# QData/FastSK

Hardware: AMD Instinct MI355X
Metric: gkm kernel build: mismatch-combos/s (higher is better)
Workload: dtype u4 count planes (v_dot8_u32_u4), u32 register sums, u64 triangle (plain stores on the first pass over reset rows, else atomics); 1 GPU; config5: synthetic DNA 100000 x 300 bp, g=12 m=8 exact, 495 combos; n_seq=100000, seq_len=300, g=12, m=8, combos=495, parallelism=single GPU

## Files before the change

### fastsk_amd/csrc/fsk_engine_dense_shift.hip

```cpp
#include "fsk_engine_internal.h"
#include "fsk_kernels_dense_shift.h"

#include <map>

using namespace fsk_detail;

namespace fsk {

#define FSK_DMA_SHIFT 1
#define FSK_DMA_KERNEL k_dense_tile_shift
#define FSK_DMA_COMPACT 0
#include "fsk_tile_kernel_dma.inc"
#undef FSK_DMA_KERNEL
#undef FSK_DMA_COMPACT
#undef FSK_DMA_SHIFT

}

namespace fsk_detail {

bool dense_shift_plan(fsk_engine* e, const int32_t* combos, int n, u64 by_overflow, uint32_t max_chain) {
    ShiftPlan& p = e->shift;
    if (!(p.by_overflow == by_overflow && p.max_chain == max_chain && (int)p.combos.size() == n && std::equal(combos, combos + n, p.combos.begin()))) {
        p = ShiftPlan();
        p.combos.assign(combos, combos + n);
        p.by_overflow = by_overflow;
        p.max_chain = max_chain;
        const int k = e->k;
        std::map<std::vector<uint8_t>, std::vector<std::pair<int, int>>> shapes;
        for (int q = 0; q < n; ++q) {
            const uint8_t* pos = &e->all_pos[(size_t)combos[q] * k];
            std::vector<uint8_t> shape(pos, pos + k);
            for (auto& x : shape) x = (uint8_t)(x - pos[0]);
            shapes[shape].push_back({(int)pos[0], q});
        }
        std::vector<std::vector<int>> chains;
        for (auto& kv : shapes) {
            auto& v = kv.second;
            std::stable_sort(v.begin(), v.end(), [](const std::pair<int, int>& a, const std::pair<int, int>& b) { return a.first < b.first; });
            for (size_t i = 0; i < v.size(); ++i) {
                if (i == 0 || v[i].first != v[i - 1].first + 1 || (max_chain != 0u && chains.back().size() >= max_chain)) chains.emplace_back();
                chains.back().push_back(v[i].second);
            }
        }
        std::stable_sort(chains.begin(), chains.end(), [](const std::vector<int>& a, const std::vector<int>& b) { return a.size() > b.size(); });
        p.n_bases = (uint32_t)chains.size();
        p.order.resize((size_t)n);
        uint32_t derived = p.n_bases;
        size_t group_begin = 0;
        for (size_t c = 0; c < chains.size(); ++c) {
            const std::vector<int>& ch = chains[c];
            const uint32_t len = (uint32_t)ch.size();
            p.order[c] = ch[0];
            if (c == 0 || chains[c - 1].size() != ch.size() || (u64)(c - group_begin) >= by_overflow) {
                p.groups.push_back(0u);
                p.groups.push_back(len);
                group_begin = c;
            }
            p.groups[p.groups.size() - 2] = (uint32_t)c + 1u;
            uint32_t lower = (uint32_t)c;
            for (uint32_t u = 1; u < len; ++u) {
                const uint32_t upper = derived++;
                p.order[upper] = ch[u];
                p.steps.push_back(upper << 16 | lower);
                p.steps.push_back(len - u);
                p.wsum += len - u;
                lower = upper;
            }
        }
    }
    return !p.steps.empty() && n <= 32768 && ((u64)2 * e->maxW + 32) * p.wsum < ((u64)1 << 31);
}

int dense_shift_edge_keys(fsk_engine* e, const uint8_t* chunk_pos, uint32_t panels_pad) {
    ShiftPlan& p = e->shift;
    const uint32_t n_steps = (uint32_t)(p.steps.size() / 2), np_seq = panels_pad * fsk::PANEL;
    FSK_HIP(e->d_shift_steps.reserve(p.steps.size()));
    FSK_HIP(e->d_edge_keys.reserve((size_t)n_steps * np_seq));
    FSK_HIP(hipMemcpyAsync(e->d_shift_steps.p, p.steps.data(), p.steps.size() * sizeof(uint32_t), hipMemcpyHostToDevice, e->stream));
    FSK_LAUNCH(fsk::k_dense_edge_keys, dim3(panels_pad, (n_steps + 3u) / 4u), dim3(256), 0, e->stream, e->view(), e->cfg.g, e->k, e->sigma, chunk_pos,
               (const uint32_t*)e->d_shift_steps.p, n_steps, np_seq, e->d_edge_keys.p);
    FSK_HIP(hipStreamSynchronize(e->stream));
    e->st.launches += 1;
    return FSK_OK;
}

int dense_shift_keymajor(fsk_engine* e, uint32_t panels_pad, int nb, uint32_t Vq8) {
    const ShiftPlan& p = e->shift;
    e->ld.shift_packed = false;
    if (e->tune.dense_shift_packed < 0 || p.max_chain != SHIFT_PACKED_CHAIN) return FSK_OK;
    const size_t plane = (size_t)panels_pad * Vq8 * fsk::PANEL * (size_t)nb;
    const size_t n_keys = (p.steps.size() / 2) * (size_t)panels_pad * fsk::PANEL;
    const size_t want = (2 * plane + n_keys) * sizeof(uint32_t);
    const char* why = nullptr;
    if (e->tune.dense_shift_plane_kb > 0 && want > (size_t)e->tune.dense_shift_plane_kb * 1024) why = "over the dense_shift_plane_kb cap";
    const size_t grow = (std::max(plane, e->d_KM.cap) - e->d_KM.cap + std::max(plane, e->d_KMH.cap) - e->d_KMH.cap +
                         std::max(n_keys, e->d_edge_offs.cap) - e->d_edge_offs.cap) * sizeof(uint32_t);
    if (!why && grow > 0) {
        size_t free_b = 0, total_b = 0;
        if (hipMemGetInfo(&free_b, &total_b) != hipSuccess) free_b = 0;
        if (grow > free_b / 2) why = "more than half of the free device memory";
        else if (e->d_KM.reserve(plane) != hipSuccess || e->d_KMH.reserve(plane) != hipSuccess || e->d_edge_offs.reserve(n_keys) != hipSuccess) {
            (void)hipGetLastError();
            e->d_KM.release(); e->d_KMH.release(); e->d_edge_offs.release();
            why = "hipMalloc failed";
        }
    }
    if (why) {
        if (e->trace())
            fprintf(stderr, "[fsk] dense shift classes: the key-major planes (%.1f MB) do not fit, %s: k_dense_shift_fix runs the corrections\n",
                    (double)want / 1e6, why);
        return FSK_OK;
    }
    const uint32_t n_pairs = panels_pad / 2u;
    const uint32_t kgrid = (uint32_t)(((size_t)n_pairs * nb * Vq8 * 16u + 255u) / 256u);
    FSK_LAUNCH(fsk::k_dense_keymajor, dim3(kgrid), dim3(256), 0, e->stream, (const uint32_t*)e->d_C4.p, n_pairs, nb, Vq8, e->d_KM.p);
    FSK_LAUNCH(fsk::k_dense_keymajor, dim3(kgrid), dim3(256), 0, e->stream, (const uint32_t*)e->d_C4H.p, n_pairs, nb, Vq8, e->d_KMH.p);
    FSK_LAUNCH(fsk::k_dense_edge_offs, dim3((uint32_t)((n_keys + 255u) / 256u)), dim3(256), 0, e->stream, (const uint16_t*)e->d_edge_keys.p, n_keys,
               e->d_edge_offs.p);
    e->st.launches += 3;
    e->ld.shift_packed = true;
    return FSK_OK;
}

int dense_shift_tiles(fsk_engine* e, u64 n_tiles, int nb, uint32_t Vq8, uint32_t nst, u64* K, int store, uint32_t panels_pad) {
    const ShiftPlan& p = e->shift;
    int slot0 = 0;
    for (size_t gi = 0; gi + 1 < p.groups.size(); gi += 2) {
        const int end = (int)p.groups[gi];
        FSK_LAUNCH(fsk::k_dense_tile_shift, dim3((uint32_t)n_tiles, 1), dim3(256), 0, e->stream, (const uint32_t*)e->d_C4.p, (const uint32_t*)e->d_C4H.p,
                   (const uint32_t*)e->d_rowmask.p, (const uint32_t*)e->d_tiletab.p, nb, Vq8, nst, (uint32_t)e->N, K, end - slot0, gi == 0 ? store : 0,
                   slot0, p.groups[gi + 1]);
        slot0 = end;
    }
    if (e->ld.shift_packed) {
        const auto k_packed = e->tune.dense_shift_inplace != 0 ? fsk::k_dense_shift_packed<true> : fsk::k_dense_shift_packed<false>;
        FSK_LAUNCH(k_packed, dim3((uint32_t)n_tiles), dim3(256), 0, e->stream, (const uint32_t*)e->d_KM.p, (const uint32_t*)e->d_KMH.p,
                   (const uint32_t*)e->d_rowmask.p, (const uint32_t*)e->d_tiletab.p, (const uint32_t*)e->d_shift_steps.p, (uint32_t)(p.steps.size() / 2),
                   (const uint32_t*)e->d_edge_offs.p, panels_pad * fsk::PANEL, nb, Vq8, p.n_bases, (uint32_t)(32u * p.wsum), (uint32_t)e->N, K);
    } else {
        FSK_LAUNCH(fsk::k_dense_shift_fix, dim3((uint32_t)n_tiles), dim3(512), 0, e->stream, (const uint32_t*)e->d_C4.p, (const uint32_t*)e->d_C4H.p,
                   (const uint32_t*)e->d_rowmask.p, (const uint32_t*)e->d_tiletab.p, (const uint32_t*)e->d_shift_steps.p, (uint32_t)(p.steps.size() / 2),
                   (const uint16_t*)e->d_edge_keys.p, panels_pad * fsk::PANEL, nb, Vq8, (uint32_t)e->N, K);
    }
    e->st.launches += (int32_t)(p.groups.size() / 2);
    return FSK_OK;
}

}
```

### fastsk_amd/csrc/fsk_engine_internal.h

```cpp
#pragma once
#include "fsk_common.h"

#include <algorithm>
#include <chrono>
#include <cmath>
#include <cstdarg>
#include <cstdio>
#include <cstdlib>
#include <cstring>
#include <string>
#include <array>
#include <atomic>
#include <thread>
#include <vector>

#include <cstdint>
#include <climits>

#include "../../include/fastsk_amd.h"
#include <condition_variable>
#include <functional>
#include <memory>
#include <mutex>

struct fsk_group;

namespace fsk_detail {

#define FSK_HIP(call)                                                                          \
    do {                                                                                       \
        hipError_t _e = (call);                                                                \
        if (_e != hipSuccess) return e->fail(FSK_EDEVICE, "%s failed: %s", #call, hipGetErrorString(_e)); \
    } while (0)

template <typename T>
struct DevBuf {
    T* p = nullptr;
    size_t cap = 0;
    DevBuf() = default;
    DevBuf(DevBuf&& o) noexcept : p(o.p), cap(o.cap) { o.p = nullptr; o.cap = 0; }
    DevBuf& operator=(DevBuf&& o) noexcept { std::swap(p, o.p); std::swap(cap, o.cap); return *this; }
    ~DevBuf() { release(); }
    hipError_t reserve(size_t n) {
        if (n <= cap) return hipSuccess;
        release();
        hipError_t r = hipMalloc((void**)&p, n * sizeof(T));
        if (r == hipSuccess) cap = n;
        return r;
    }
    void release() {
        if (p) (void)hipFree(p);
        p = nullptr;
        cap = 0;
    }
};

template <typename T>
struct PinnedBuf {
    T* p = nullptr;
    size_t cap = 0;
    PinnedBuf() = default;
    PinnedBuf(PinnedBuf&& o) noexcept : p(o.p), cap(o.cap) { o.p = nullptr; o.cap = 0; }
    PinnedBuf& operator=(PinnedBuf&& o) noexcept { std::swap(p, o.p); std::swap(cap, o.cap); return *this; }
    ~PinnedBuf() { release(); }
    hipError_t reserve(size_t n, size_t slack = 0) {
        if (n <= cap) return hipSuccess;
        release();
        hipError_t r = hipHostMalloc((void**)&p, (n + slack) * sizeof(T));
        if (r == hipSuccess) cap = n + slack;
        return r;
    }
    void release() {
        if (p) (void)hipHostFree(p);
        p = nullptr;
        cap = 0;
    }
};

template <typename H, hipError_t (*Create)(H*, unsigned), hipError_t (*Destroy)(H)>
struct Handle {
    H h = nullptr;
    Handle() = default;
    Handle(Handle&& o) noexcept : h(o.h) { o.h = nullptr; }
    Handle& operator=(Handle&& o) noexcept { std::swap(h, o.h); return *this; }
    ~Handle() { if (h) (void)Destroy(h); }
    hipError_t create(unsigned flags) { return h ? hipSuccess : Create(&h, flags); }
    operator H() const { return h; }
};
using Stream = Handle<hipStream_t, hipStreamCreateWithFlags, hipStreamDestroy>;
using Event = Handle<hipEvent_t, hipEventCreateWithFlags, hipEventDestroy>;

struct DeviceScope {
    int prev = -1, dev;
    hipError_t err = hipSuccess;
    explicit DeviceScope(int d) : dev(d) {
        if (hipGetDevice(&prev) != hipSuccess) prev = -1;
        if (prev != dev) err = hipSetDevice(dev);
    }
    ~DeviceScope() {
        if (prev >= 0 && prev != dev) (void)hipSetDevice(prev);
    }
    DeviceScope(const DeviceScope&) = delete;
    DeviceScope& operator=(const DeviceScope&) = delete;
};
#define FSK_ON_DEVICE(e)                                                                      \
    DeviceScope fsk_on_device_((e)->cfg.device);                                             \
    if (fsk_on_device_.err != hipSuccess)                                                    \
        return (e)->fail(FSK_EDEVICE, "hipSetDevice(%d) failed: %s", (e)->cfg.device, hipGetErrorString(fsk_on_device_.err))

}

using fsk_detail::DevBuf;
using fsk_detail::PinnedBuf;
using fsk_detail::Stream;
using fsk_detail::Event;

#define FSK_TUNING_KEYS(X)                                                                                                          \
    X(trace, 0, 0, 1, "stderr: the tuning in force, where the host time of a load and of a variance-mode call goes")                 \
    X(profile, -1, -1, 2, "fsk_config.profile from here on (-1: as the engine was created)")                                          \
    X(compact, -1, -1, 1, "dense: key compaction off / on whatever the alphabet says (-1: a rare symbol decides)")                   \
    X(compact_rare, -1, -1, 1, "dense: keys that occur from the places of the rare symbols (1) or a marking pass over every window (0)") \
    X(tile_splits, 0, 0, 4096, "dense: combo splits per tile (0: by the size of the launch)")                                        \
    X(dense_small, 0, 0, 1, "dense: 1 = a split tile launch (small N) leaves its sums as 32-bit staging blocks that k_dense_widen adds into K (0: one 64-bit atomic a cell and split — measured faster: the atomics drain under other workgroups' dot products)")                                        \
    X(dense_shift, 0, -1, 1, "dense: one weighted Gram product per chain of shifted combinations, the other members by edge lookups (fsk_engine_dense_shift.hip) — 1 = whenever the call is eligible, -1 = never (0: when eligible, tile_splits = 0 and the launch has 16384 tiles or more, the size from which a tile has one workgroup anyway)") \
    X(dense_shift_packed, 0, -1, 0, "dense, shift classes: the derived steps from key-major planes, eight cells an LDS read (k_dense_keymajor, k_dense_shift_packed; chains cut at nine members) — 0 = whenever the shift path runs and the planes fit, -1 = never: k_dense_shift_fix on the count panels") \
    X(dense_shift_inplace, 1, 0, 1, "dense, shift classes: k_dense_shift_packed stages a chain's first planes and makes every further step's in LDS, one nibble up and one down a sequence (a step that meets a count above 15 in its tile, and the step behind it, are staged) — 0 = every step staged") \
    X(dense_shift_plane_kb, 0, 0, (int64_t)1 << 40, "dense, shift classes: the key-major planes and offsets may take this many KiB at most (0: half of the free memory; tests: the planes do not fit)") \
    X(dense_chunk, 0, 0, 1 << 24, "dense: cap of the count kernel's staging chunk, in windows (0: none)")                             \
    X(variance_dense_slots, 1, 0, 1, "variance mode, dense: 0 = zero fill + k_welford per iteration instead of storing slot triangles") \
    X(var_slots16, 1, 0, 1, "variance mode, sparse: 0 = u32 slot triangles from the start")                                          \
    X(sparse_global, 0, 0, 1, "sparse: every += as a 64-bit atomicAdd (k_sx_emit<DIRECT>) whatever N is")                             \
    X(sparse_unpacked, 0, 0, 1, "sparse: entries in the general 8 + 4 (+ 4) byte format whatever N is")                               \
    X(sparse_pairs, 1, 0, 1, "sparse: 0 = every update word 32 bits wide (1: unit products of clean runs travel two to a word)")      \
    X(sparse_sync, 0, 0, 1, "sparse: wait for every batch's word count and size its stream exactly")                                 \
    X(sparse_hint, 1, 0, 1, "sparse: 0 = the words per record of the previous set of sequences are never kept as a hint")             \
    X(sparse_exact_lanes, 0, 0, 2, "sparse: the batches of an exact accumulate never (1) / always (2) in two lanes (0: from six batches on)") \
    X(sparse_batch_records, 0, 0, (int64_t)1 << 31, "sparse: records per batch at most (0: 2^27)")                                   \
    X(guard_cap, 0, 0, (int64_t)1 << 40, "sparse: pretend the stream buffer holds this many words (0: its real size)")                \
    X(list_max_words, 0, 0, (int64_t)1 << 31, "sparse: update words of one batch beyond which its pairs go to K with atomics (0: 2^31)") \
    X(seg_scan_chunked, 0, 0, 1, "sparse: the three-launch segment scan whatever the tile count")                                    \
    X(extract_slots, 0, 0, 4, "sparse: slots per k_sx_extract_win workgroup, 1 or 4 (0: by the size of the launch)")                  \
    X(sparse_form, 0, 0, 3, "sparse: the update stage — 1 = owner bands whenever they exist, 2 = two-level blocks, 3 = 64-bit atomics (0: bands up to four LDS rounds a band, blocks beyond)") \
    X(blocks_sub_shift, 14, 4, 14, "sparse, blocks: log2 of the cells one k_sxb_consume workgroup sums in LDS (tests: small blocks on small inputs)") \
    X(blocks_max_bands, 512, 2, 512, "sparse, blocks: bands of one pass at most (tests: several passes on small inputs)")            \
    X(blocks_band_shift_max, 23, 4, 23, "sparse, blocks: log2 of a band's cells at most (tests)")                                    \
    X(blocks_pass_words, 0, 0, (int64_t)1 << 32, "sparse, blocks: update words of one pass at most (0: 2^31)")                       \
    X(sparse_desc, 0, -1, 1, "sparse, owner bands and two-level blocks: entries of many partners leave k_sx_emit as descriptors (one an entry; blocks: one per sub-band its partners fall into) that k_sx_consume / k_sxb_consume expand in LDS — 1 = always, -1 = never (0: once a batch of these sequences has shown sparse_desc_from pairs per record)") \
    X(sparse_desc_blocks, 1, 0, 1, "sparse, two-level blocks: 0 = never descriptors there (1: as sparse_desc says — one record per sub-band an entry's partners fall into)") \
    X(sparse_desc_cols, 1, 0, 3, "sparse, descriptors: where the partners are read from — 0 = the entries themselves; 1 = a column array (sequence id | multiplicity, 4 bytes) beside 8-byte entries, the entries themselves when they are packed (measured: 2-byte columns beside packed entries are no faster, 0.88 against 0.84 s in the large-g regime; 4-byte columns beside 8-byte entries 4.69 -> 4.44 ms a combo at N = 100k); tests: 2 = 4-byte columns always, 3 = 2-byte columns when N < 32768") \
    X(sparse_desc_min, 16, 1, 48, "sparse, descriptors: entries of more partners than this become descriptors (48: everything k_sx_emit does not bin in LDS; measured, large-g regime: 48 0.92 s, 32 0.85, 16 0.83-0.85, 8 0.88, 4 0.90)") \
    X(sparse_desc_from, 12, 1, 1 << 20, "sparse, descriptors: the pairs per sort record of a batch from which on the following batches use them (sparse_desc = 0)") \
    X(sparse_parts_target, 0, 0, 1 << 30, "sparse, owner bands: words of one k_sx_consume part (0: four LDS rounds' worth at least, 1/1024 of the batch's words; tests: several parts a band on small inputs)") \
    X(sparse_desc_parts, 2048, 1, 1 << 16, "sparse, descriptors: parts (k_sx_consume workgroups) the bands' streams are cut into, about") \
    X(sparse_share, 0, -1, 254, "sparse: leading kept positions sorted once per group of consecutive combos that share them (0: by cost; -1: never); batches of more than 16 slots only (smaller ones read their positions by id), and never when the presort's scratch passes a quarter of the free memory") \
    X(seed_splitmix, 0, 0, 1, "approx modes: 1 = fsk_set_seed draws the engine's older splitmix64 Fisher-Yates order (0: the reference's std::shuffle of minstd_rand0)") \
    X(mismatch_order, 0, 0, 1, "mismatch-weighted mode: 1 = the levels run from m = d down to 0 (0: from 0 up to d)")                   \
    X(collective, 0, 0, 2, "fsk_create_multi: FSK_COLL_* when fsk_config.collective is FSK_COLL_AUTO")                                \
    X(deadline_ms, 120000, -1, 86400000, "fsk_create_multi: the fail-fast bound when fsk_config.deadline_ms is 0 (negative: none)")   \
    X(svm_wg_max, 8192, 0, 8192, "fsk_svm_train: up to this many training rows the solver is one workgroup with alpha, G and y in LDS (k_svm_wg); beyond, two launches an iteration (k_svm_select_i / k_svm_select_j); 0 = always those") \
    X(svm_chunk, 256, 1, 65536, "fsk_svm_train: iterations enqueued between two reads of the solver's status record (k_svm_wg: iterations a launch)") \
    X(rows_tile, FSK_ROWS_TILE, FSK_ROWS_TILE, FSK_ROWS_TILE, "fsk_rows_build, read-only: the edge T of k_rows_syrk's tile of the rows kernel (compiled in)") \
    X(rows_panel, FSK_ROWS_PANEL, FSK_ROWS_PANEL, FSK_ROWS_PANEL, "fsk_rows_build, read-only: the consecutive train columns P a panel of k_rows_syrk stages in LDS (compiled in)") \
    FSK_TUNING_TEST_KEYS(X)
#ifdef FSK_TEST_HOOKS
#define FSK_TUNING_TEST_KEYS(X)                                            \
    X(fault_kind, 0, 0, 3, "test hook: 1 = host sleep, 2 = device spin before a band's collective; 3 = host sleep after the variance chains")   \
    X(fault_rank, -1, -1, 15, "test hook: the engine that is late")        \
    X(fault_band, -1, -1, 63, "test hook: before this band's collective")  \
    X(fault_ms, 0, 0, 60000, "test hook: by this many milliseconds")
#else
#define FSK_TUNING_TEST_KEYS(X)
#endif
struct fsk_tuning {
#define FSK_X(name, def, lo, hi, doc) int64_t name = (def);
    FSK_TUNING_KEYS(FSK_X)
#undef FSK_X
};

struct SxScratch {
    DevBuf<unsigned char> d_keys[2];
    DevBuf<uint32_t> d_blockhist, d_totals, d_tile_ent, d_ebase, d_Pk, d_Tk, d_ucount, d_uchunk, d_utot, d_list_off, d_ulist, d_part_base;
    DevBuf<u64> d_tile_stat;
    DevBuf<uint32_t> d_segc;
    DevBuf<int> d_tile_lrh, d_tile_rs, d_tile_lth, d_tile_ts;
    DevBuf<uint2> d_E;
    DevBuf<u64> d_sxstat;
    DevBuf<uint32_t> d_group_of, d_group_head, d_winp;
    DevBuf<unsigned char> d_part;
    DevBuf<uint32_t> d_ulist2, d_subcnt, d_suboff, d_subcur;
    DevBuf<uint32_t> d_dsubcnt, d_dsuboff, d_dsubcur;
    DevBuf<uint32_t> d_cols;
};

struct ShiftPlan {
    std::vector<int32_t> combos;
    u64 by_overflow = 0;
    std::vector<int32_t> order;
    std::vector<uint32_t> groups, steps;
    uint32_t n_bases = 0;
    uint32_t max_chain = 0;
    u64 wsum = 0;
};

struct SvmCvState {
    bool valid = false;
    std::vector<double> oof;
    std::vector<fsk_svm_cv_score> scores;
    std::vector<fsk_svm_cv_problem> problems;
    std::vector<double> alpha;
    std::vector<uint32_t> idx;
    std::vector<u64> st_off, idx_off;
    fsk_svm_cv_info info{};
    DevBuf<double> d_alpha, d_G, d_krow, d_coef, d_rho, d_oof;
    DevBuf<uint32_t> d_idx;
    DevBuf<int32_t> d_fold;
    DevBuf<signed char> d_y;
    DevBuf<unsigned char> d_prob, d_rec;
};

struct SvmState {
    bool valid = false;
    SvmCvState cv;
    std::vector<double> alpha;
    std::vector<signed char> y;
    double rho = 0;
    int kernel = 0;
    double w_pos = 1.0, w_neg = 1.0;
    double C = 0, eps = 0;
    int64_t max_iter = 0;
    SvmCvState cal;
    bool platt_valid = false;
    fsk_svm_platt_info platt{};
    fsk_svm_info info{};
    DevBuf<double> d_alpha, d_G, d_krow, d_coef, d_out;
    DevBuf<signed char> d_y;
    DevBuf<unsigned char> d_rec;
};

struct RowsState {
    bool valid = false;
    DevBuf<double> d_L, d_diag;
    fsk_rows_info info{};
    void drop() { valid = false; d_L.release(); d_diag.release(); }
};

struct fsk_engine {
    Stream stream;
    Stream lane_stream;
    Stream chain_stream;
    fsk_config cfg{};
    int cfg_profile0 = 0;
    fsk_tuning tune{};
    std::string err;
    int k = 0;
    int64_t ncomb = 0;
    Event ev0, ev1;
    Event ev_out, ev_in;
    fsk_group* group = nullptr;
    bool store_next = false;
    PinnedBuf<uint32_t> h_stage;
    bool stage_in_flight = false;
    PinnedBuf<double> h_prod;

    struct Loaded {
        bool featseq_ready = false;
        bool rare_ready = false;
        bool prep_valid = false, prep_overflow = false, prep_shift = false, shift_packed = false;
        uint32_t prep_chain = 0;
        double vc_sum = 0, vc_n = 0;
        bool u_known = false, u_pending = false;
        u64 u_value = 0, u_extra = 0;
        struct SxDefer { bool active = false; u64 cap = 0, nrec = 0; } sx_defer[8];
        int64_t lazy_lo = -1, lazy_hi = -1;
        std::vector<double> stdevs;
        u64 sx_passes = 0;
        int sx_form_used = -1;
        bool sx_desc_used = false;
        int sx_share_used = 0;
        uint32_t sx_share_groups = 0;
    } ld;

    bool loaded = false, finalized = false, result_f64 = false;
    int64_t N = 0, n_train = 0, n_test = 0, nfeat = 0, pairs = 0;
    uint32_t sigma = 0, Lmax = 0, Lmin = 0, maxW = 0, Vq = 0, n_panels = 0;
    int bits = 0;
    u64 V = 0;
    int path = 0;
    DevBuf<uint32_t> d_words, d_wstart, d_len, d_fstart, d_featseq;
    DevBuf<uint32_t> d_win;
    int win_words = 0;
    std::vector<uint32_t> h_len, h_fstart;
    std::vector<int32_t> rc_tokens, rc_comps;
    bool revcomp = false;
    uint32_t maxW1 = 0;
    DevBuf<uint16_t> d_comp;
    std::vector<int32_t> wild_tokens;
    bool wild = false;
    DevBuf<uint32_t> d_vbits, d_vstart, d_fwin;
    std::vector<uint8_t> cw_profile;
    bool cw = false, fwin_on = false;
    uint32_t cw_n = 0;
    DevBuf<uint8_t> d_cw;

    std::vector<uint64_t> mm_c;
    std::vector<int64_t> mm_a;
    bool mm_plain = false;
    DevBuf<u64> mm_scratch;
    std::vector<int64_t> mm_ran_a;
    std::vector<int32_t> mm_ran_path;
    std::vector<double> mm_ran_level_ms, mm_ran_fold_ms;
    bool mm_on() const { return !mm_c.empty(); }

    std::vector<uint8_t> all_pos;
    DevBuf<uint8_t> d_pos, d_allpos;
    bool allpos_ready = false;
    std::vector<int32_t> order;
    bool order_set = false;
    uint64_t seed = 0;

    u64* d_K = nullptr;
    bool K_owned = false;
    int64_t bound_cells = 0;
    DevBuf<u64> K_store;
    DevBuf<double> d_Kf64, d_Khat, d_prod, d_diag, d_stage, d_bsum;
    DevBuf<unsigned char> d_seqblk;
    DevBuf<u64> d_stage_u64, d_Kslots;
    DevBuf<int64_t> d_cell_idx;

    DevBuf<uint32_t> d_C4, d_C4H, d_rowmask, d_flag;
    DevBuf<uint32_t> d_stage32;
    DevBuf<uint32_t> d_keybits;
    DevBuf<uint16_t> d_lut, d_vc;
    bool compact = false;
    bool compact_rare = false;
    uint32_t rare_mask = 0, rare_places = 0;
    DevBuf<u64> d_rare;
    DevBuf<uint32_t> d_rare_n, d_common;
    std::vector<uint16_t> h_vc_cache;
    DevBuf<uint32_t> d_tiletab;
    uint32_t tab_t0 = 0, tab_t1 = 0, tab_n = 0;
    uint32_t tab_ftt = 0xffffffffu;
    std::vector<int32_t> prep_combos;
    ShiftPlan shift;
    DevBuf<uint32_t> d_shift_steps;
    DevBuf<uint16_t> d_edge_keys;
    DevBuf<uint32_t> d_KM, d_KMH, d_edge_offs;
    SxScratch sxs[2];
    Event ev_lane[4];
    DevBuf<uint32_t> d_owner_r0;
    DevBuf<u64> d_U;
    std::vector<uint32_t> h_owner_r0;
    uint32_t n_owners = 0, sx_rounds = 1, sx_cap = 0;
    uint32_t sx_rounds_slot = 1, sx_cap_slot = 0;
    int sx_pb = 16, sx_sb = 1, sx_keybits = 1, sx_own_shift = 13;
    int sx_symbits = 0;
    bool sx_lists = false, owner_ready = false;
    int n_cu = 256;
    int sx_form = 0;
    DevBuf<uint32_t> d_blk_r0;
    bool sx_pairs_asked = true;
    bool sx_pairs = false;
    int64_t owner_N = -1;
    DevBuf<u64> d_U2;
    std::vector<int32_t> u_combos;
    PinnedBuf<unsigned char> h_sx_pos;
    PinnedBuf<u64> h_sx_stat;
    PinnedBuf<unsigned char> h_sx_head_pos;
    PinnedBuf<u64> h_sx_head_stat;
    bool sx_slot16 = false;
    bool sx_slot16_used = false;
    bool slots16_ok = true;
    PinnedBuf<uint32_t> h_sx_head_flag;
    uint32_t* sx_ovf_now = nullptr;
    int sx_last_lane = 0;
    u64 sx_shape[4] = {0, 0, 0, 0};
    double sx_ppr = 0;
    double sx_wpr = 0;
    u64 sx_words_of(u64 nrec) const { return (u64)(sx_wpr * (double)nrec) + 1; }
    void sx_saw(u64 words, u64 nrec) { if (nrec) sx_wpr = std::max(sx_wpr, std::max(1e-9, (double)words / (double)nrec)); }
    bool sx_desc_now() const { return tune.sparse_desc > 0 || (tune.sparse_desc == 0 && sx_ppr >= (double)tune.sparse_desc_from); }
    void sx_saw_pairs(u64 pairs, u64 nrec) {
        if (!nrec) return;
        const bool was = sx_desc_now();
        sx_ppr = std::max(sx_ppr, (double)pairs / (double)nrec);
        if (!was && sx_desc_now()) sx_wpr = 0;
    }
    u64 sx_redone = 0;
    bool sx_redoing = false;
    bool sx_exactly() const { return tune.sparse_sync != 0 || sx_redoing; }
    u64 sx_max_words() const { return tune.list_max_words > 0 ? std::min<u64>((u64)1 << 31, (u64)tune.list_max_words) : (u64)1 << 31; }
    bool trace() const { return tune.trace != 0; }

    fsk_stats st{};
    SvmState svm;
    RowsState rows;

    int fail(int code, const char* fmt, ...) {
        char buf[512];
        va_list ap;
        va_start(ap, fmt);
        vsnprintf(buf, sizeof buf, fmt, ap);
        va_end(ap);
        err = buf;
        return code;
    }
    fsk::SeqView view() const {
        return fsk::SeqView{d_words.p, d_wstart.p, d_len.p, (uint32_t)N, bits};
    }
    struct LazyTime { Event a, b; double* acc; };
    std::vector<LazyTime> lazy_pending;
    std::vector<Event> lazy_free;
    Event lazy_open;
    bool profile_sync() const { return cfg.profile == 1; }
    Event lazy_event() {
        Event ev;
        if (!lazy_free.empty()) { ev = std::move(lazy_free.back()); lazy_free.pop_back(); }
        else if (ev.create(0) != hipSuccess) (void)hipGetLastError();
        return ev;
    }
    void lazy_done(LazyTime& t, bool reached) {
        float ms = 0;
        if (reached && hipEventElapsedTime(&ms, t.a, t.b) == hipSuccess) *t.acc += ms;
        lazy_free.push_back(std::move(t.a));
        lazy_free.push_back(std::move(t.b));
    }
    void harvest_times() {
        for (LazyTime& t : lazy_pending) lazy_done(t, hipEventSynchronize(t.b) == hipSuccess);
        lazy_pending.clear();
    }
    void harvest_finished() {
        size_t keep = 0;
        for (LazyTime& t : lazy_pending) {
            if (hipEventQuery(t.b) == hipSuccess) lazy_done(t, true);
            else {
                (void)hipGetLastError();
                lazy_pending[keep++] = std::move(t);
            }
        }
        lazy_pending.resize(keep);
    }
    void lazy_interval(Event a, Event b, double* acc) {
        if (!a || !b) return;
        lazy_pending.push_back(LazyTime{std::move(a), std::move(b), acc});
        if (lazy_pending.size() >= 512 && lazy_pending.size() % 128 == 0) harvest_finished();
    }
    void tic(hipStream_t s = nullptr) {
        if (cfg.profile == 1) (void)hipEventRecord(ev0, s ? s : stream);
        else if (cfg.profile == 2) {
            if (lazy_open) lazy_free.push_back(std::move(lazy_open));
            lazy_open = lazy_event();
            if (lazy_open) (void)hipEventRecord(lazy_open, s ? s : stream);
        }
    }
    void toc(double* acc, hipStream_t s = nullptr) {
        if (cfg.profile == 1) {
            (void)hipEventRecord(ev1, s ? s : stream);
            (void)hipEventSynchronize(ev1);
            float ms = 0;
            (void)hipEventElapsedTime(&ms, ev0, ev1);
            *acc += ms;
        } else if (cfg.profile == 2 && lazy_open) {
            Event b = lazy_event();
            if (b) (void)hipEventRecord(b, s ? s : stream);
            lazy_interval(std::move(lazy_open), std::move(b), acc);
        }
    }
};

namespace fsk_detail {

constexpr size_t LDS_BUDGET = 150 * 1024;
constexpr u64 DENSE_MAX_KEYS = 16384;
constexpr size_t SPARSE_MAX_RECORDS = 1u << 27;
constexpr int FSK_RETRY_UNGROUPED = 1;

int tuning_set(fsk_tuning& t, const char* key, int64_t value, std::string& err);
int tuning_parse(fsk_tuning& t, const char* text, std::string& err);
std::string tuning_in_force(const fsk_tuning& t);
void set_create_error(const std::string& msg);
int64_t n_choose_k(int n, int k);
int materialise_zero(fsk_engine* e);
bool lazy_zero_possible(const fsk_engine* e);
int do_accumulate(fsk_engine* e, const int32_t* combos, int n, u64* K, int64_t row0 = 0, int64_t row1 = -1, u64 slot_stride = 0,
                  int defer = -1);
int make_diag(fsk_engine* e);
int launch_triangle(fsk_engine* e, u64 c0, u64 cnt, double* dst);
int rows_build(fsk_engine* e);
void default_order(fsk_engine* e);
void libstdcxx_shuffle_order(uint64_t seed, int64_t n, int32_t* out);

struct DensePlan { uint32_t CH = 0, Vcq = 0; size_t lds = 0; };
DensePlan dense_plan(uint32_t maxW, int g, uint32_t Vq, size_t extra = 0);
size_t dense_mode_lds(const fsk_engine* e);
int fetch_pending_u(fsk_engine* e);
int accumulate_dense(fsk_engine* e, const int32_t* combos, int n, u64* K, int64_t row0, int64_t row1);
size_t dense_small_stage_bytes(u64 n_tiles, int n_splits);
int dense_tile_small(fsk_engine* e, bool compact, u64 n_tiles, int n_splits, int nb, uint32_t Vq8, uint32_t nst, u64* K, int slots_per_split);

constexpr uint32_t SHIFT_PACKED_CHAIN = 9;
bool dense_shift_plan(fsk_engine* e, const int32_t* combos, int n, u64 by_overflow, uint32_t max_chain);
int dense_shift_edge_keys(fsk_engine* e, const uint8_t* chunk_pos, uint32_t panels_pad);
int dense_shift_keymajor(fsk_engine* e, uint32_t panels_pad, int nb, uint32_t Vq8);
int dense_shift_tiles(fsk_engine* e, u64 n_tiles, int nb, uint32_t Vq8, uint32_t nst, u64* K, int store, uint32_t panels_pad);

inline int sx_lane_of(const fsk_engine* e, int defer) { return (defer >= 0 && !e->profile_sync()) ? (defer & 1) : 0; }
struct SxPass { int64_t ra = 0, rb = 0; int t = 14, sub_shift = 14, pb = 8; uint32_t n_owners = 0, submax = 0, own_base = 0; std::vector<uint32_t> r0; };
bool blocks_plan_pass(fsk_engine* e, int64_t ra, int64_t rb, SxPass* out);
void plan_owner_bands(fsk_engine* e);
bool sx_harvest(fsk_engine* e, int slot);
int accumulate_sparse(fsk_engine* e, const int32_t* combos, int n, u64* K, int64_t row0, int64_t row1, u64 slot_stride = 0,
                      int defer = -1);

int run_variance_mode(fsk_engine* e, int T, int chain_first = 0, int chain_step = 1);

int one_load_sequences(fsk_engine* e, const int32_t* tokens, const int64_t* offsets, int64_t n_train, int64_t n_test);
int one_reset_counts(fsk_engine* e);
int one_reset_counts_rows(fsk_engine* e, int64_t row_begin, int64_t row_end);
int one_accumulate_rows(fsk_engine* e, const int32_t* combos, int32_t n, int64_t row_begin, int64_t row_end);
int one_synchronize(fsk_engine* e);
int one_finalize(fsk_engine* e);
int one_set_combo_order(fsk_engine* e, const int32_t* order, int32_t n);
int one_set_complement(fsk_engine* e, const int32_t* tokens, const int32_t* complements, int32_t n);
int one_set_wildcards(fsk_engine* e, const int32_t* tokens, int32_t n);
int one_set_center_weights(fsk_engine* e, const uint32_t* w, int32_t n);
int one_get_stats(fsk_engine* e, fsk_stats* out);
void one_destroy(fsk_engine* e);
void skip_variance_combos(fsk_engine* e, std::vector<int32_t>& used);
int approx_chains(const fsk_engine* e);
int mismatch_solve(int g, const uint64_t* c, int n, std::vector<int64_t>& a, std::string& why);
int mismatch_compute(fsk_engine* e, const int32_t* tokens, const int64_t* offsets, int64_t n_train, int64_t n_test);

int group_load_sequences(fsk_engine* e, const int32_t* tokens, const int64_t* offsets, int64_t n_train, int64_t n_test);
int group_reset_counts(fsk_engine* e, int64_t row_begin, int64_t row_end);
int group_accumulate(fsk_engine* e, const int32_t* combos, int32_t n);
int group_synchronize(fsk_engine* e);
int group_finalize(fsk_engine* e);
int group_compute(fsk_engine* e, const int32_t* tokens, const int64_t* offsets, int64_t n_train, int64_t n_test);
int group_set_combo_order(fsk_engine* e, const int32_t* order, int32_t n);
int group_set_seed(fsk_engine* e, uint64_t seed);
int group_set_complement(fsk_engine* e, const int32_t* tokens, const int32_t* complements, int32_t n);
int group_set_wildcards(fsk_engine* e, const int32_t* tokens, int32_t n);
int group_set_center_weights(fsk_engine* e, const uint32_t* w, int32_t n);
int group_get_stats(fsk_engine* e, fsk_stats* out);
int group_set_skip_test_block(fsk_engine* e, int32_t skip);
int group_set_tuning(fsk_engine* e, const char* key, int64_t value, std::string& err);
void group_set_profile(fsk_engine* e, int profile);
void group_destroy(fsk_engine* e);
void group_note_bound_counts(fsk_engine* e);

}
```

### fastsk_amd/csrc/fsk_tile_kernel_dma.inc

```
#ifndef FSK_DMA_STAGE32
#define FSK_DMA_STAGE32 0
#endif
#ifndef FSK_DMA_SHIFT
#define FSK_DMA_SHIFT 0
#endif
__global__ __launch_bounds__(256, 4) void FSK_DMA_KERNEL(const uint32_t* C4, const uint32_t* C4H, const uint32_t* rowmask,
                                                        const uint32_t* tile_tab, int n_slots, uint32_t Vq8, uint32_t nst,
                                                        uint32_t N,
#if FSK_DMA_STAGE32
                                                        uint32_t* stage32,
#else
                                                        u64* K,
#endif
                                                        int slots_per_split, int store
#if FSK_DMA_COMPACT
                                                        , const uint16_t* vc
#endif
#if FSK_DMA_SHIFT
                                                        , int slot0, uint32_t weight
#endif
) {
    constexpr int MAXF = 4;
#if FSK_DMA_COMPACT
    constexpr int MASK_WORDS = 960;
    constexpr int ROW_SLOTS = 64;
#else
    constexpr int MASK_WORDS = 1024;
#endif
    constexpr int DMA_ROWS = 16;
    constexpr int PBUF = 4 * DMA_ROWS * PANEL;
    __shared__ __attribute__((aligned(1024))) uint32_t P[2 * PBUF + 2 * MAXF * TILE];
    __shared__ uint32_t smask[1024];
    uint32_t* const AsH = P + 2 * PBUF;
    uint32_t* const BsH = P + 2 * PBUF + MAXF * TILE;
    const int tid = threadIdx.x, ty = tid >> 4, tx = tid & 15;
    const uint32_t tile = tile_tab[blockIdx.x];
    const uint32_t ti = tile >> 16, tj = tile & 0xffffu;
#if FSK_DMA_SHIFT
    const int s0 = slot0;
#else
    const int s0 = blockIdx.y * slots_per_split;
#endif
    const int s1 = s0 + slots_per_split < n_slots ? s0 + slots_per_split : n_slots;
#if !FSK_DMA_STAGE32
    if (s0 >= s1) return;
#endif
    const size_t slot_stride = (size_t)Vq8 * PANEL;
    const size_t panel_stride = (size_t)n_slots * slot_stride;

    uint32_t acc[8][8];
#pragma unroll
    for (int a = 0; a < 8; ++a)
#pragma unroll
        for (int b = 0; b < 8; ++b) acc[a][b] = 0u;

#define FSK_PANEL_OF(which) (((which) < 2u ? ti : tj) * 2u + ((which) & 1u))
    const uint32_t lane_off_b = (((uint32_t)tid >> 4) * PANEL + ((uint32_t)tid & 15u) * 4u) * 4u;
    const fsk_hw::lds_addr_t lds_wave = fsk_hw::lds_address(P) + (uint32_t)__builtin_amdgcn_readfirstlane(tid >> 6) * 1024u;
    auto load_stage = [&](int buf, int slot, uint32_t kq0, uint32_t rows) {
        const size_t so = (size_t)slot * slot_stride + (size_t)kq0 * PANEL;
        const uint32_t left = (uint32_t)__builtin_amdgcn_readfirstlane((int)(rows - kq0));
        const uint32_t bytes = (left < (uint32_t)DMA_ROWS ? left : (uint32_t)DMA_ROWS) * PANEL * 4u;
#pragma unroll
        for (int w = 0; w < 4; ++w)
            fsk_hw::panel_rows_to_lds(C4 + FSK_PANEL_OF((uint32_t)w) * panel_stride + so, bytes,
                                      lds_wave + (uint32_t)(buf * PBUF + w * DMA_ROWS * PANEL) * 4u, lane_off_b);
    };
    auto wait_loads = [&]() { fsk_hw::wait_panel_rows(); };
    auto fetch_hi = [&](int slot, uint32_t kq0, uint32_t m) -> uint4 {
        const uint32_t f = (uint32_t)tid >> 6;
        for (uint32_t q = 0; q < f; ++q) m &= m - 1u;
        uint4 h = make_uint4(0u, 0u, 0u, 0u);
        if (m) {
            const uint32_t row = kq0 + (uint32_t)__ffs((int)m) - 1u;
            const uint32_t within = (uint32_t)tid & 63u, which = within >> 4, r4 = within & 15u;
            h = *reinterpret_cast<const uint4*>(C4H + FSK_PANEL_OF(which) * panel_stride + (size_t)slot * slot_stride +
                                                (size_t)row * PANEL + r4 * 4u);
        }
        return h;
    };
    auto park_hi = [&](const uint4& h) {
        const uint32_t f = (uint32_t)tid >> 6, within = (uint32_t)tid & 63u, which = within >> 4, r4 = within & 15u;
        uint32_t* dst = (which < 2 ? AsH : BsH) + f * TILE + (which & 1u) * PANEL + r4 * 4u;
        *reinterpret_cast<uint4*>(dst) = h;
    };
#if FSK_DMA_COMPACT
    auto fix_row = [&](const uint32_t* pb, uint32_t r, uint32_t f, bool hasA, bool hasB) {
        auto frag = [&](const uint32_t* p0, const uint32_t* p1, int t, uint32_t (&v)[8]) {
            const uint4 x0 = *reinterpret_cast<const uint4*>(&p0[t * 4]);
            const uint4 x1 = *reinterpret_cast<const uint4*>(&p1[t * 4]);
            v[0] = x0.x; v[1] = x0.y; v[2] = x0.z; v[3] = x0.w; v[4] = x1.x; v[5] = x1.y; v[6] = x1.z; v[7] = x1.w;
        };
        const uint32_t* alo = pb + r * PANEL;
        const uint32_t* blo = pb + 2 * DMA_ROWS * PANEL + r * PANEL;
        uint32_t p[8], q[8];
        if (hasA) {
            frag(&AsH[f * TILE], &AsH[f * TILE + PANEL], ty, p);
            frag(blo, blo + DMA_ROWS * PANEL, tx, q);
#pragma unroll
            for (int a = 0; a < 8; ++a)
#pragma unroll
                for (int b = 0; b < 8; ++b) acc[a][b] += __builtin_amdgcn_udot8(p[a], q[b], 0u, false) << 4;
        }
        if (hasB) {
            frag(alo, alo + DMA_ROWS * PANEL, ty, p);
            frag(&BsH[f * TILE], &BsH[f * TILE + PANEL], tx, q);
#pragma unroll
            for (int a = 0; a < 8; ++a)
#pragma unroll
                for (int b = 0; b < 8; ++b) acc[a][b] += __builtin_amdgcn_udot8(p[a], q[b], 0u, false) << 4;
        }
        if (hasA && hasB) {
            frag(&AsH[f * TILE], &AsH[f * TILE + PANEL], ty, p);
            frag(&BsH[f * TILE], &BsH[f * TILE + PANEL], tx, q);
#pragma unroll
            for (int a = 0; a < 8; ++a)
#pragma unroll
                for (int b = 0; b < 8; ++b) acc[a][b] += __builtin_amdgcn_udot8(p[a], q[b], 0u, false) << 8;
        }
    };
#else
    auto fix_row = [&](const uint32_t* pb, uint32_t r, uint32_t f, bool, bool) {
        const uint4 b0 = *reinterpret_cast<const uint4*>(&pb[2 * DMA_ROWS * PANEL + r * PANEL + tx * 4]);
        const uint4 b1 = *reinterpret_cast<const uint4*>(&pb[3 * DMA_ROWS * PANEL + r * PANEL + tx * 4]);
        const uint4 d0 = *reinterpret_cast<const uint4*>(&BsH[f * TILE + tx * 4]);
        const uint4 d1 = *reinterpret_cast<const uint4*>(&BsH[f * TILE + PANEL + tx * 4]);
        const uint32_t blo[8] = {b0.x, b0.y, b0.z, b0.w, b1.x, b1.y, b1.z, b1.w};
        const uint32_t bhi[8] = {d0.x, d0.y, d0.z, d0.w, d1.x, d1.y, d1.z, d1.w};
#pragma unroll
        for (int a = 0; a < 8; ++a) {
            const uint32_t alo = pb[(a >> 2) * DMA_ROWS * PANEL + r * PANEL + ty * 4 + (a & 3)];
            const uint32_t ahi = AsH[f * TILE + (a >> 2) * PANEL + ty * 4 + (a & 3)];
#pragma unroll
            for (int b = 0; b < 8; ++b) {
                uint32_t t = __builtin_amdgcn_udot8(alo, bhi[b], 0u, false);
                t = __builtin_amdgcn_udot8(ahi, blo[b], t, false);
                const uint32_t u = __builtin_amdgcn_udot8(ahi, bhi[b], 0u, false);
                acc[a][b] += 16u * t + 256u * u;
            }
        }
    };
#endif

#if FSK_DMA_COMPACT
    constexpr uint32_t MW = 2u;
    int chunk_slots = (int)(MASK_WORDS / (MW * nst)) > 0 ? (int)(MASK_WORDS / (MW * nst)) : 1;
    if (chunk_slots > ROW_SLOTS) chunk_slots = ROW_SLOTS;
#define FSK_ROWS_OF(sl) smask[MASK_WORDS + (uint32_t)((sl) - c0)]
#else
    const int chunk_slots = (int)(MASK_WORDS / nst) > 0 ? (int)(MASK_WORDS / nst) : 1;
#define FSK_ROWS_OF(sl) Vq8
#endif
    for (int c0 = s0; c0 < s1; c0 += chunk_slots) {
        const int c1 = c0 + chunk_slots < s1 ? c0 + chunk_slots : s1;
        __syncthreads();
        for (uint32_t i = tid; i < (uint32_t)(c1 - c0) * nst; i += 256) {
            const uint32_t sl = (uint32_t)c0 + i / nst, st = i % nst;
            const size_t a = ((size_t)(ti * 2u) * n_slots + sl) * nst + st, b = ((size_t)(tj * 2u) * n_slots + sl) * nst + st;
            const size_t np = (size_t)n_slots * nst;
#if FSK_DMA_COMPACT
            smask[2u * i] = rowmask[a] | rowmask[a + np];
            smask[2u * i + 1u] = rowmask[b] | rowmask[b + np];
#else
            smask[i] = rowmask[a] | rowmask[a + np] | rowmask[b] | rowmask[b + np];
#endif
        }
#if FSK_DMA_COMPACT
        if (tid < c1 - c0) smask[MASK_WORDS + tid] = ((uint32_t)vc[c0 + tid] + 7u) >> 3;
        __syncthreads();
#endif
        int slot = c0;
#if FSK_DMA_COMPACT
        while (slot < c1 && FSK_ROWS_OF(slot) == 0u) ++slot;
        if (slot >= c1) continue;
#endif
        uint32_t kq0 = 0;
        int buf = 0;
        load_stage(buf, slot, kq0, FSK_ROWS_OF(slot));
        wait_loads();
        __syncthreads();
        while (slot < c1) {
            const uint32_t rows_s = __builtin_amdgcn_readfirstlane(FSK_ROWS_OF(slot));
            int nslot = slot;
            uint32_t nkq0 = kq0 + DMA_ROWS;
            if (nkq0 >= rows_s) {
                nslot = slot + 1;
                nkq0 = 0;
#if FSK_DMA_COMPACT
                while (nslot < c1 && FSK_ROWS_OF(nslot) == 0u) ++nslot;
#endif
            }
#if FSK_DMA_COMPACT
            const uint32_t mi = 2u * ((uint32_t)(slot - c0) * nst + (kq0 >> 5));
            const uint32_t maskA = (__builtin_amdgcn_readfirstlane(smask[mi]) >> (kq0 & 16u)) & 0xffffu;
            const uint32_t maskB = (__builtin_amdgcn_readfirstlane(smask[mi + 1u]) >> (kq0 & 16u)) & 0xffffu;
            const uint32_t mask = maskA | maskB;
#else
            const uint32_t mword = __builtin_amdgcn_readfirstlane(smask[(uint32_t)(slot - c0) * nst + (kq0 >> 5)]);
            const uint32_t mask = (mword >> (kq0 & 16u)) & 0xffffu;
#endif
            uint4 hreg = make_uint4(0u, 0u, 0u, 0u);
            if (mask) hreg = fetch_hi(slot, kq0, mask);
            if (nslot < c1) load_stage(buf ^ 1, nslot, nkq0, FSK_ROWS_OF(nslot));
            const uint32_t rows_left = rows_s - kq0;
            const int nkq = rows_left < (uint32_t)DMA_ROWS ? (int)rows_left : DMA_ROWS;
            const uint32_t* pb = P + buf * PBUF;
#pragma unroll 2
            for (int kq = 0; kq < nkq; ++kq) {
                const uint4 a0 = *reinterpret_cast<const uint4*>(&pb[kq * PANEL + ty * 4]);
                const uint4 a1 = *reinterpret_cast<const uint4*>(&pb[DMA_ROWS * PANEL + kq * PANEL + ty * 4]);
                const uint4 b0 = *reinterpret_cast<const uint4*>(&pb[2 * DMA_ROWS * PANEL + kq * PANEL + tx * 4]);
                const uint4 b1 = *reinterpret_cast<const uint4*>(&pb[3 * DMA_ROWS * PANEL + kq * PANEL + tx * 4]);
                const uint32_t av[8] = {a0.x, a0.y, a0.z, a0.w, a1.x, a1.y, a1.z, a1.w};
                const uint32_t bv[8] = {b0.x, b0.y, b0.z, b0.w, b1.x, b1.y, b1.z, b1.w};
#pragma unroll
                for (int a = 0; a < 8; ++a)
#pragma unroll
                    for (int b = 0; b < 8; ++b) acc[a][b] = __builtin_amdgcn_udot8(av[a], bv[b], acc[a][b], false);
            }
            if (mask) {
                uint32_t m = mask;
                bool first = true;
                while (m) {
                    if (!first) {
                        hreg = fetch_hi(slot, kq0, m);
                        __syncthreads();
                    }
                    park_hi(hreg);
                    __syncthreads();
                    for (uint32_t f = 0; f < (uint32_t)MAXF && m; ++f) {
                        const uint32_t r = (uint32_t)__ffs((int)m) - 1u;
#if FSK_DMA_COMPACT
                        fix_row(pb, r, f, (maskA >> r) & 1u, (maskB >> r) & 1u);
#else
                        fix_row(pb, r, f, true, true);
#endif
                        m &= m - 1u;
                    }
                    first = false;
                }
            }
            wait_loads();
            __syncthreads();
            slot = nslot;
            kq0 = nkq0;
            buf ^= 1;
        }
    }
#undef FSK_PANEL_OF
#undef FSK_ROWS_OF
#if FSK_DMA_STAGE32
    {
        uint32_t* blk = stage32 + ((size_t)blockIdx.y * gridDim.x + blockIdx.x) * (size_t)(TILE * TILE);
#pragma unroll
        for (int a = 0; a < 8; ++a)
#pragma unroll
            for (int b = 0; b < 8; ++b) blk[(a * 8 + b) * 256 + tid] = acc[a][b];
    }
#else
#pragma unroll
    for (int a = 0; a < 8; ++a) {
        const u64 i = (u64)ti * TILE + tile_index((uint32_t)ty, (uint32_t)a);
        if (i >= N) continue;
#pragma unroll
        for (int b = 0; b < 8; ++b) {
            const u64 j = (u64)tj * TILE + tile_index((uint32_t)tx, (uint32_t)b);
            if (j <= i && (store || acc[a][b] != 0u)) {
                const uint32_t lo = fsk_hw::vgpr_copy(acc[a][b]);
#if FSK_DMA_SHIFT
                if (store) K[tri_index(i, j)] = (u64)lo * weight;
                else atomicAdd(&K[tri_index(i, j)], (u64)lo * weight);
#else
                if (store) K[tri_index(i, j)] = (u64)lo;
                else atomicAdd(&K[tri_index(i, j)], (u64)lo);
#endif
            }
        }
    }
#endif
}
```

Measured before the change: 435.8 combos/s.

## Fuse all chain-length group base products into one launch with incremental weighted flushes

Instead of one k_dense_tile_shift launch per chain-length group, each of which re-accumulates from its own slot range and writes the triangle, a new kernel variant walks all base slots in one launch. At each group end it flushes the running accumulator into K, weighted by the difference in chain length between consecutive groups, and does not clear it. Because group lengths fall, this telescoping sum reproduces the per-group weights. It saves repeated launch overhead and re-reading of tiles. The cost is that every group boundary inside the slot loop now does a full triangle flush, with atomics after the first, and a new host-side group_steps table.

```diff
diff --git a/fastsk_amd/csrc/fsk_engine_dense_shift.hip b/fastsk_amd/csrc/fsk_engine_dense_shift.hip
--- a/fastsk_amd/csrc/fsk_engine_dense_shift.hip
+++ b/fastsk_amd/csrc/fsk_engine_dense_shift.hip
@@ -10,6 +10,12 @@
 #define FSK_DMA_SHIFT 1
 #define FSK_DMA_KERNEL k_dense_tile_shift
 #define FSK_DMA_COMPACT 0
+#include "fsk_tile_kernel_dma.inc"
+#undef FSK_DMA_KERNEL
+#undef FSK_DMA_SHIFT
+
+#define FSK_DMA_SHIFT 2
+#define FSK_DMA_KERNEL k_dense_tile_shift_all
 #include "fsk_tile_kernel_dma.inc"
 #undef FSK_DMA_KERNEL
 #undef FSK_DMA_COMPACT
@@ -68,6 +74,16 @@
                 lower = upper;
             }
         }
+        bool falling = true;
+        for (size_t gi = 2; gi + 1 < p.groups.size(); gi += 2) falling = falling && p.groups[gi + 1] < p.groups[gi - 1];
+        if (falling) {
+            for (size_t gi = 0; gi + 1 < p.groups.size(); gi += 2) {
+                p.group_steps.push_back(p.groups[gi]);
+                p.group_steps.push_back(p.groups[gi + 1] - (gi + 3 < p.groups.size() ? p.groups[gi + 3] : 0u));
+            }
+            p.group_steps.push_back(0xffffffffu);
+            p.group_steps.push_back(0u);
+        }
     }
     return !p.steps.empty() && n <= 32768 && ((u64)2 * e->maxW + 32) * p.wsum < ((u64)1 << 31);
 }
@@ -75,9 +91,12 @@
 int dense_shift_edge_keys(fsk_engine* e, const uint8_t* chunk_pos, uint32_t panels_pad) {
     ShiftPlan& p = e->shift;
     const uint32_t n_steps = (uint32_t)(p.steps.size() / 2), np_seq = panels_pad * fsk::PANEL;
-    FSK_HIP(e->d_shift_steps.reserve(p.steps.size()));
+    FSK_HIP(e->d_shift_steps.reserve(p.steps.size() + p.group_steps.size()));
     FSK_HIP(e->d_edge_keys.reserve((size_t)n_steps * np_seq));
     FSK_HIP(hipMemcpyAsync(e->d_shift_steps.p, p.steps.data(), p.steps.size() * sizeof(uint32_t), hipMemcpyHostToDevice, e->stream));
+    if (!p.group_steps.empty())
+        FSK_HIP(hipMemcpyAsync(e->d_shift_steps.p + p.steps.size(), p.group_steps.data(), p.group_steps.size() * sizeof(uint32_t), hipMemcpyHostToDevice,
+                               e->stream));
     FSK_LAUNCH(fsk::k_dense_edge_keys, dim3(panels_pad, (n_steps + 3u) / 4u), dim3(256), 0, e->stream, e->view(), e->cfg.g, e->k, e->sigma, chunk_pos,
                (const uint32_t*)e->d_shift_steps.p, n_steps, np_seq, e->d_edge_keys.p);
     FSK_HIP(hipStreamSynchronize(e->stream));
@@ -125,13 +144,23 @@
 
 int dense_shift_tiles(fsk_engine* e, u64 n_tiles, int nb, uint32_t Vq8, uint32_t nst, u64* K, int store, uint32_t panels_pad) {
     const ShiftPlan& p = e->shift;
-    int slot0 = 0;
-    for (size_t gi = 0; gi + 1 < p.groups.size(); gi += 2) {
-        const int end = (int)p.groups[gi];
-        FSK_LAUNCH(fsk::k_dense_tile_shift, dim3((uint32_t)n_tiles, 1), dim3(256), 0, e->stream, (const uint32_t*)e->d_C4.p, (const uint32_t*)e->d_C4H.p,
-                   (const uint32_t*)e->d_rowmask.p, (const uint32_t*)e->d_tiletab.p, nb, Vq8, nst, (uint32_t)e->N, K, end - slot0, gi == 0 ? store : 0,
-                   slot0, p.groups[gi + 1]);
-        slot0 = end;
+    const bool one_launch = !p.group_steps.empty() && (e->tune.dense_shift_one_launch > 0 ||
+                                                       (e->tune.dense_shift_one_launch == 0 && e->tune.tile_splits == 0 && n_tiles >= 16384));
+    int base_launches = 1;
+    if (one_launch) {
+        FSK_LAUNCH(fsk::k_dense_tile_shift_all, dim3((uint32_t)n_tiles, 1), dim3(256), 0, e->stream, (const uint32_t*)e->d_C4.p,
+                   (const uint32_t*)e->d_C4H.p, (const uint32_t*)e->d_rowmask.p, (const uint32_t*)e->d_tiletab.p, nb, Vq8, nst, (uint32_t)e->N, K,
+                   (int)p.n_bases, store, (const uint32_t*)e->d_shift_steps.p + p.steps.size());
+    } else {
+        base_launches = (int)(p.groups.size() / 2);
+        int slot0 = 0;
+        for (size_t gi = 0; gi + 1 < p.groups.size(); gi += 2) {
+            const int end = (int)p.groups[gi];
+            FSK_LAUNCH(fsk::k_dense_tile_shift, dim3((uint32_t)n_tiles, 1), dim3(256), 0, e->stream, (const uint32_t*)e->d_C4.p,
+                       (const uint32_t*)e->d_C4H.p, (const uint32_t*)e->d_rowmask.p, (const uint32_t*)e->d_tiletab.p, nb, Vq8, nst, (uint32_t)e->N, K,
+                       end - slot0, gi == 0 ? store : 0, slot0, p.groups[gi + 1]);
+            slot0 = end;
+        }
     }
     if (e->ld.shift_packed) {
         const auto k_packed = e->tune.dense_shift_inplace != 0 ? fsk::k_dense_shift_packed<true> : fsk::k_dense_shift_packed<false>;
@@ -143,7 +172,7 @@
                    (const uint32_t*)e->d_rowmask.p, (const uint32_t*)e->d_tiletab.p, (const uint32_t*)e->d_shift_steps.p, (uint32_t)(p.steps.size() / 2),
                    (const uint16_t*)e->d_edge_keys.p, panels_pad * fsk::PANEL, nb, Vq8, (uint32_t)e->N, K);
     }
-    e->st.launches += (int32_t)(p.groups.size() / 2);
+    e->st.launches += (int32_t)base_launches;
     return FSK_OK;
 }
 
diff --git a/fastsk_amd/csrc/fsk_engine_internal.h b/fastsk_amd/csrc/fsk_engine_internal.h
--- a/fastsk_amd/csrc/fsk_engine_internal.h
+++ b/fastsk_amd/csrc/fsk_engine_internal.h
@@ -125,6 +125,7 @@
     X(dense_shift, 0, -1, 1, "dense: one weighted Gram product per chain of shifted combinations, the other members by edge lookups (fsk_engine_dense_shift.hip) — 1 = whenever the call is eligible, -1 = never (0: when eligible, tile_splits = 0 and the launch has 16384 tiles or more, the size from which a tile has one workgroup anyway)") \
     X(dense_shift_packed, 0, -1, 0, "dense, shift classes: the derived steps from key-major planes, eight cells an LDS read (k_dense_keymajor, k_dense_shift_packed; chains cut at nine members) — 0 = whenever the shift path runs and the planes fit, -1 = never: k_dense_shift_fix on the count panels") \
     X(dense_shift_inplace, 1, 0, 1, "dense, shift classes: k_dense_shift_packed stages a chain's first planes and makes every further step's in LDS, one nibble up and one down a sequence (a step that meets a count above 15 in its tile, and the step behind it, are staged) — 0 = every step staged") \
+    X(dense_shift_one_launch, 0, -1, 1, "dense, shift classes: every chain-length group of the base products in ONE launch that flushes at the group ends without clearing (k_dense_tile_shift_all) — 1 = whenever the shift path runs, -1 = never: one k_dense_tile_shift launch a group (0: where the shift path runs by its own default rule, tile_splits = 0 and 16384 tiles or more)") \
     X(dense_shift_plane_kb, 0, 0, (int64_t)1 << 40, "dense, shift classes: the key-major planes and offsets may take this many KiB at most (0: half of the free memory; tests: the planes do not fit)") \
     X(dense_chunk, 0, 0, 1 << 24, "dense: cap of the count kernel's staging chunk, in windows (0: none)")                             \
     X(variance_dense_slots, 1, 0, 1, "variance mode, dense: 0 = zero fill + k_welford per iteration instead of storing slot triangles") \
@@ -196,7 +197,7 @@
     std::vector<int32_t> combos;
     u64 by_overflow = 0;
     std::vector<int32_t> order;
-    std::vector<uint32_t> groups, steps;
+    std::vector<uint32_t> groups, steps, group_steps;
     uint32_t n_bases = 0;
     uint32_t max_chain = 0;
     u64 wsum = 0;
diff --git a/fastsk_amd/csrc/fsk_tile_kernel_dma.inc b/fastsk_amd/csrc/fsk_tile_kernel_dma.inc
--- a/fastsk_amd/csrc/fsk_tile_kernel_dma.inc
+++ b/fastsk_amd/csrc/fsk_tile_kernel_dma.inc
@@ -16,8 +16,10 @@
 #if FSK_DMA_COMPACT
                                                         , const uint16_t* vc
 #endif
-#if FSK_DMA_SHIFT
+#if FSK_DMA_SHIFT == 1
                                                         , int slot0, uint32_t weight
+#elif FSK_DMA_SHIFT == 2
+                                                        , const uint32_t* groups
 #endif
 ) {
     constexpr int MAXF = 4;
@@ -36,8 +38,10 @@
     const int tid = threadIdx.x, ty = tid >> 4, tx = tid & 15;
     const uint32_t tile = tile_tab[blockIdx.x];
     const uint32_t ti = tile >> 16, tj = tile & 0xffffu;
-#if FSK_DMA_SHIFT
+#if FSK_DMA_SHIFT == 1
     const int s0 = slot0;
+#elif FSK_DMA_SHIFT == 2
+    const int s0 = 0;
 #else
     const int s0 = blockIdx.y * slots_per_split;
 #endif
@@ -150,6 +154,29 @@
 #else
     const int chunk_slots = (int)(MASK_WORDS / nst) > 0 ? (int)(MASK_WORDS / nst) : 1;
 #define FSK_ROWS_OF(sl) Vq8
+#endif
+#if FSK_DMA_SHIFT == 2
+    int g_end = __builtin_amdgcn_readfirstlane((int)groups[0]);
+    uint32_t g_step = (uint32_t)__builtin_amdgcn_readfirstlane((int)groups[1]);
+    int g_at = 0;
+    auto flush_group = [&](uint32_t step, bool st) {
+        const uint32_t t = fsk_hw::vgpr_copy((uint32_t)tid);
+        const uint32_t fy = t >> 4, fx = t & 15u;
+#pragma unroll
+        for (int a = 0; a < 8; ++a) {
+            const u64 i = (u64)ti * TILE + tile_index(fy, (uint32_t)a);
+            if (i >= N) continue;
+#pragma unroll
+            for (int b = 0; b < 8; ++b) {
+                const u64 j = (u64)tj * TILE + tile_index(fx, (uint32_t)b);
+                if (j <= i && (st || acc[a][b] != 0u)) {
+                    const uint32_t lo = fsk_hw::vgpr_copy(acc[a][b]);
+                    if (st) K[tri_index(i, j)] = (u64)lo * step;
+                    else atomicAdd(&K[tri_index(i, j)], (u64)lo * step);
+                }
+            }
+        }
+    };
 #endif
     for (int c0 = s0; c0 < s1; c0 += chunk_slots) {
         const int c1 = c0 + chunk_slots < s1 ? c0 + chunk_slots : s1;
@@ -240,6 +267,14 @@
                     first = false;
                 }
             }
+#if FSK_DMA_SHIFT == 2
+            if (nslot != slot && nslot == g_end) {
+                flush_group(g_step, store != 0 && g_at == 0);
+                ++g_at;
+                g_end = __builtin_amdgcn_readfirstlane((int)groups[2 * g_at]);
+                g_step = (uint32_t)__builtin_amdgcn_readfirstlane((int)groups[2 * g_at + 1]);
+            }
+#endif
             wait_loads();
             __syncthreads();
             slot = nslot;
@@ -257,7 +292,7 @@
 #pragma unroll
             for (int b = 0; b < 8; ++b) blk[(a * 8 + b) * 256 + tid] = acc[a][b];
     }
-#else
+#elif FSK_DMA_SHIFT != 2
 #pragma unroll
     for (int a = 0; a < 8; ++a) {
         const u64 i = (u64)ti * TILE + tile_index((uint32_t)ty, (uint32_t)a);
@@ -267,7 +302,7 @@
             const u64 j = (u64)tj * TILE + tile_index((uint32_t)tx, (uint32_t)b);
             if (j <= i && (store || acc[a][b] != 0u)) {
                 const uint32_t lo = fsk_hw::vgpr_copy(acc[a][b]);
-#if FSK_DMA_SHIFT
+#if FSK_DMA_SHIFT == 1
                 if (store) K[tri_index(i, j)] = (u64)lo * weight;
                 else atomicAdd(&K[tri_index(i, j)], (u64)lo * weight);
 #else
```

Measured after the change: 453.0 combos/s, median of 6. +3.9%, better.
